# mcahny/vps

Hardware: AMD Instinct MI355X
Metric: frames/sec FuseTrack 1024x2048 (higher is better)
Workload: dtype f32-grade: f16x3 split operands (fp16 pair with scaled residual, 22 significand bits) on MFMA, f32 accumulate

## Files before the change

vps_amd/csrc/conv_mfma.hip:

```cpp
#include "conv_common.h"

namespace {
template <int TM, int TN, int WAVES_M, int WAVES_N, bool DEFORM>
__global__ __launch_bounds__(256, 2)
void conv_mfma_f32_kernel(const vps_conv_desc d, const int M, const int tiles_m, const int tiles_n,
                          const int ksteps_per_split) {
    constexpr int BN = WAVES_N * TN * 32;
    static_assert(WAVES_M * TM * 32 == BM, "block M tile must be 128");
    static_assert(WAVES_M * WAVES_N == 4, "4 wavefronts per block");
    constexpr int NB = BN / 32;

    __shared__ __attribute__((aligned(16))) float As[BM * LDS_LD];
    __shared__ __attribute__((aligned(16))) float Bs[BN * LDS_LD];

    const int t = threadIdx.x;
    int swz = xcd_swizzle(blockIdx.x, gridDim.x);
    int tile_n, tile_m, cls, split;
    decode_tile(d, swz, tiles_n, tiles_m, tile_n, tile_m, cls, split);

    const int py = cls / d.os_x, px = cls - py * d.os_x;
    const int pad_y = d.pad_y[py], pad_x = d.pad_x[px];
    const float* __restrict__ wcls = d.w + (size_t)cls * d.cout_pad * d.kpad;

    const int H = d.H, W = d.W, KH = d.KH, KW = d.KW, cin_pad = d.cin_pad;
    const int k4 = t & 7;
    const int r0 = t >> 3;

    RowInfo ri[4];
#pragma unroll
    for (int i = 0; i < 4; ++i) {
        const int m = tile_m * BM + r0 + 32 * i;
        if (m < M) {
            const int qx = m % d.Qw;
            const int tq = m / d.Qw;
            const int qy = tq % d.Qh;
            const int n = tq / d.Qh;
            ri[i].iy0 = qy * d.stride - pad_y;
            ri[i].ix0 = qx * d.stride - pad_x;
            ri[i].pixbase = n * H * W;
            ri[i].moff = m;
        } else {
            ri[i].iy0 = -(1 << 24);
            ri[i].ix0 = 0;
            ri[i].pixbase = 0;
            ri[i].moff = -1;
        }
    }

    const int kstep0 = split * ksteps_per_split;
    int nsteps = d.kpad / BK - kstep0;
    if (nsteps > ksteps_per_split) nsteps = ksteps_per_split;
    const int korder = d.korder, ntap = KH * KW;
    int ky, kx, ci;
    if (korder == 0) {
        const int kk = kstep0 * BK + k4 * 4;
        const int tap = kk / cin_pad;
        ci = kk - tap * cin_pad;
        ky = tap / KW;
        kx = tap - ky * KW;
    } else {
        const int chunk = kstep0 / ntap, tap = kstep0 - chunk * ntap;
        ci = chunk * BK + k4 * 4;
        ky = tap / KW;
        kx = tap - ky * KW;
    }
    const float* __restrict__ wrow = wcls + (size_t)(tile_n * BN + r0) * d.kpad + (size_t)kstep0 * BK + k4 * 4;

    f32x4 areg[4];
    unsigned aok = 0;
    f32x4 breg[NB];
    f32x4 dcv[DEFORM ? 4 : 1][4];
    float dcw[DEFORM ? 4 : 1][4];

    auto load_tiles = [&](int step) {
        const bool kval = ky < KH && ci < cin_pad;
        if constexpr (!DEFORM) {
#pragma unroll
            for (int i = 0; i < 4; ++i) {
                const int iy = ri[i].iy0 + ky, ix = ri[i].ix0 + kx;
                const bool ok = kval && (unsigned)iy < (unsigned)H && (unsigned)ix < (unsigned)W;
                const int pix = ri[i].pixbase + (ok ? iy * W + ix : 0);
                areg[i] = *reinterpret_cast<const f32x4*>(d.in + ((size_t)pix * d.in_ld + d.in_coff + (ok ? ci : 0)));
                aok = (aok & ~(1u << i)) | ((ok ? 1u : 0u) << i);
            }
        } else {
            const int tap = ky * KW + kx;
#pragma unroll
            for (int i = 0; i < 4; ++i) {
                const bool act = kval && ri[i].moff >= 0;
                const float* op = d.offset + (size_t)(act ? ri[i].moff : 0) * d.off_ld + 2 * min(tap, KH * KW - 1);
                const float h_im = (float)(ri[i].iy0 + ky) + op[0];
                const float w_im = (float)(ri[i].ix0 + kx) + op[1];
                const bool inside = act && h_im > -1.f && w_im > -1.f && h_im < (float)H && w_im < (float)W;
                const float hf = floorf(h_im), wf = floorf(w_im);
                const int h_low = inside ? (int)hf : 0, w_low = inside ? (int)wf : 0;
                const int h_high = h_low + 1, w_high = w_low + 1;
                const float lh = h_im - hf, lw = w_im - wf;
                const float hh = 1.f - lh, hw = 1.f - lw;
                const bool hl = inside && h_low >= 0, hhv = inside && h_high <= H - 1;
                const bool wl = w_low >= 0, whv = w_high <= W - 1;
                dcw[i][0] = (hl && wl) ? hh * hw : 0.f;
                dcw[i][1] = (hl && whv) ? hh * lw : 0.f;
                dcw[i][2] = (hhv && wl) ? lh * hw : 0.f;
                dcw[i][3] = (hhv && whv) ? lh * lw : 0.f;
                const int hlc = min(max(h_low, 0), H - 1), hhc = min(max(h_high, 0), H - 1);
                const int wlc = min(max(w_low, 0), W - 1), whc = min(max(w_high, 0), W - 1);
                const float* base = d.in + (size_t)ri[i].pixbase * d.in_ld + d.in_coff + ci;
                dcv[i][0] = *reinterpret_cast<const f32x4*>(base + (size_t)(hlc * W + wlc) * d.in_ld);
                dcv[i][1] = *reinterpret_cast<const f32x4*>(base + (size_t)(hlc * W + whc) * d.in_ld);
                dcv[i][2] = *reinterpret_cast<const f32x4*>(base + (size_t)(hhc * W + wlc) * d.in_ld);
                dcv[i][3] = *reinterpret_cast<const f32x4*>(base + (size_t)(hhc * W + whc) * d.in_ld);
            }
        }
#pragma unroll
        for (int j = 0; j < NB; ++j)
            breg[j] = *reinterpret_cast<const f32x4*>(wrow + (size_t)(32 * j) * d.kpad + (size_t)step * BK);
        if (korder == 0) {
            ci += BK;
            while (ci >= cin_pad) {
                ci -= cin_pad;
                if (++kx == KW) { kx = 0; ++ky; }
            }
        } else if (++kx == KW) {
            kx = 0;
            if (++ky == KH) { ky = 0; ci += BK; }
        }
    };

    auto store_tiles = [&]() {
#pragma unroll
        for (int i = 0; i < 4; ++i) {
            f32x4 v;
            if constexpr (DEFORM) {
                v = dcw[i][0] * dcv[i][0] + dcw[i][1] * dcv[i][1] + dcw[i][2] * dcv[i][2] + dcw[i][3] * dcv[i][3];
            } else {
                const f32x4 z = {0.f, 0.f, 0.f, 0.f};
                v = ((aok >> i) & 1u) ? areg[i] : z;
            }
            *reinterpret_cast<f32x4*>(&As[(r0 + 32 * i) * LDS_LD + k4 * 4]) = v;
        }
#pragma unroll
        for (int j = 0; j < NB; ++j)
            *reinterpret_cast<f32x4*>(&Bs[(r0 + 32 * j) * LDS_LD + k4 * 4]) = breg[j];
    };

    const int lane = t & 63, wave = t >> 6;
    const int wm = wave / WAVES_N, wn = wave - wm * WAVES_N;
    const int frag_off = (lane & 31) * LDS_LD + (lane >> 5) * 4;

    f32x16 acc[TM][TN];
#pragma unroll
    for (int a = 0; a < TM; ++a)
#pragma unroll
        for (int b = 0; b < TN; ++b)
#pragma unroll
            for (int r = 0; r < 16; ++r) acc[a][b][r] = 0.f;

    if (nsteps > 0) {
        load_tiles(0);
        store_tiles();
    }
    __syncthreads();

    for (int step = 0; step < nsteps; ++step) {
        const bool more = step + 1 < nsteps;
        if (more) load_tiles(step + 1);
#pragma unroll
        for (int kg = 0; kg < 4; ++kg) {
            f32x4 af[TM], bf[TN];
#pragma unroll
            for (int a = 0; a < TM; ++a)
                af[a] = *reinterpret_cast<const f32x4*>(&As[(wm * TM * 32 + a * 32) * LDS_LD + frag_off + kg * 8]);
#pragma unroll
            for (int b = 0; b < TN; ++b)
                bf[b] = *reinterpret_cast<const f32x4*>(&Bs[(wn * TN * 32 + b * 32) * LDS_LD + frag_off + kg * 8]);
#pragma unroll
            for (int j = 0; j < 4; ++j)
#pragma unroll
                for (int a = 0; a < TM; ++a)
#pragma unroll
                    for (int b = 0; b < TN; ++b)
                        acc[a][b] = __builtin_amdgcn_mfma_f32_32x32x2f32(bf[b][j], af[a][j], acc[a][b], 0, 0, 0);
        }
        __syncthreads();
        if (more) {
            store_tiles();
            __syncthreads();
        }
    }

    conv_epilogue<TM, TN, BN>(d, acc, M, tile_m, tile_n, cls, split, py, px, wm, wn, lane, (cls * tiles_m + tile_m) * tiles_n + tile_n);
}

template <int TM, int TN, int WAVES_M, int WAVES_N, int MODE, bool TAPMAJOR, bool DEFORM = false>
__global__ __launch_bounds__(256, (TN >= 4 ? 1 : 2))
void conv_mfma_bf16p_kernel(const vps_conv_desc d, const int M, const int tiles_m, const int tiles_n,
                            const int ksteps_per_split) {
    constexpr int BN = WAVES_N * TN * 32;
    static_assert(WAVES_M * TM * 32 == BM, "block M tile must be 128");
    static_assert(WAVES_M * WAVES_N == 4, "4 wavefronts per block");
    typedef Split<MODE> SM;
    typedef typename SM::elem elem_t;
    typedef vec8<elem_t> x8;
    typedef vec4<elem_t> x4;
    constexpr int NSA = SM::NSA, NSB = SM::NSB;
    constexpr int ABUF = NSA * BM * LDS_LDH;

    __shared__ __attribute__((aligned(16))) elem_t As[2 * ABUF];
    constexpr int DTAP = 9;
    __shared__ __attribute__((aligned(16))) float cw[DEFORM ? BM * DTAP * 4 : 4];
    __shared__ __attribute__((aligned(8))) unsigned short cc[DEFORM ? BM * DTAP * 4 : 4];
    static_assert(!(DEFORM && TAPMAJOR), "deformable layers use the chunk-major order");

    const int t = threadIdx.x;
    int swz = xcd_swizzle(blockIdx.x, gridDim.x);
    int tile_n, tile_m, cls, split;
    decode_tile(d, swz, tiles_n, tiles_m, tile_n, tile_m, cls, split);

    const int py = cls / d.os_x, px = cls - py * d.os_x;
    const int pad_y = d.pad_y[py], pad_x = d.pad_x[px];
    const int H = d.H, W = d.W, KH = d.KH, KW = d.KW, cin_pad = d.cin_pad;
    const int k4 = t & 7;
    const int r0 = t >> 3;

    RowInfo ri[4];
#pragma unroll
    for (int i = 0; i < 4; ++i) {
        const int m = tile_m * BM + r0 + 32 * i;
        if (m < M) {
            const int qx = m % d.Qw;
            const int tq = m / d.Qw;
            const int qy = tq % d.Qh;
            const int n = tq / d.Qh;
            ri[i].iy0 = qy * d.stride - pad_y;
            ri[i].ix0 = qx * d.stride - pad_x;
            ri[i].pixbase = n * H * W;
        } else {
            ri[i].iy0 = -(1 << 24);
            ri[i].ix0 = 0;
            ri[i].pixbase = 0;
        }
        ri[i].moff = m;
    }

    const int kstep0 = split * ksteps_per_split;
    int nsteps = d.kpad / BK - kstep0;
    if (nsteps > ksteps_per_split) nsteps = ksteps_per_split;
    const int korder = d.korder, ntap = KH * KW;
    int ky = 0, kx = 0, chunk = 0, astep = kstep0;
    if constexpr (!TAPMAJOR) {
        chunk = kstep0 / ntap;
        const int tap = kstep0 - chunk * ntap;
        ky = tap / KW;
        kx = tap - ky * KW;
    }
    (void)korder;

    const int lane = t & 63;
    const int wave = __builtin_amdgcn_readfirstlane(t >> 6);
    const int wm = wave / WAVES_N, wn = wave - wm * WAVES_N;
    const int nbt = d.cout_pad >> 5, kst = d.kpad >> 4;
    const size_t wplane = (size_t)d.nclass * nbt * kst * 512;
    const __amdgpu_buffer_rsrc_t wrsrc = make_rsrc(d.w_split, (unsigned)(wplane * NSB * sizeof(elem_t)));
    const unsigned wbase = (unsigned)((((size_t)(cls * nbt + tile_n * (BN / 32) + wn * TN) * kst + 2 * (size_t)kstep0) * 512) * sizeof(elem_t));
    const unsigned wlane = (unsigned)lane * 16u;
    const unsigned in_bytes = (unsigned)((size_t)d.N * H * W * d.in_ld * sizeof(float));
    const __amdgpu_buffer_rsrc_t arsrc = make_rsrc(d.in, in_bytes);
    const unsigned ld4 = (unsigned)d.in_ld * 4u;
    const unsigned acoff = (unsigned)(d.in_coff + k4 * 4) * 4u;
    unsigned rowoff[4];
#pragma unroll
    for (int i = 0; i < 4; ++i) rowoff[i] = (unsigned)(ri[i].pixbase + ri[i].iy0 * W + ri[i].ix0) * ld4 + acoff;

    f32x4 areg[DEFORM ? 1 : 2][4];
    f32x4 dcv[DEFORM ? 4 : 1][4];
    float dcw[DEFORM ? 4 : 1][4];
    x8 bnext[2][NSB][TN];
    float amax = 0.f;

    auto load_A = [&](const int slot) {
        int kyc, kxc, chunk_of_step = 0;
        unsigned stepoff;
        bool kv;
        if constexpr (!TAPMAJOR) {
            kyc = ky; kxc = kx;
            kv = chunk * BK + k4 * 4 < cin_pad;
            chunk_of_step = chunk;
            stepoff = (unsigned)(kyc * W + kxc) * ld4 + (unsigned)chunk * (BK * 4u);
            if (++kx == KW) {
                kx = 0;
                if (++ky == KH) { ky = 0; ++chunk; }
            }
        } else {
            const int kk = astep * BK + k4 * 4;
            const int tap = kk / cin_pad;
            const int cic = kk - tap * cin_pad;
            kyc = tap / KW;
            kxc = tap - kyc * KW;
            kv = tap < ntap;
            stepoff = (unsigned)(kyc * W + kxc) * ld4 + (unsigned)(cic - k4 * 4) * 4u;
        }
        ++astep;
        if constexpr (DEFORM) {
            const int tap = min(kyc * KW + kxc, DTAP - 1);
            const unsigned choff = acoff + (unsigned)chunk_of_step * (BK * 4u);
#pragma unroll
            for (int i = 0; i < 4; ++i) {
                const int e = ((r0 + 32 * i) * DTAP + tap) * 4;
                const f32x4 w4 = *reinterpret_cast<const f32x4*>(&cw[e]);
                const vec4<unsigned short> c4 = *reinterpret_cast<const vec4<unsigned short>*>(&cc[e]);
                dcw[i][0] = w4[0]; dcw[i][1] = w4[1]; dcw[i][2] = w4[2]; dcw[i][3] = w4[3];
                const unsigned pb = (unsigned)ri[i].pixbase;
                const unsigned o00 = (pb + (unsigned)c4[0] * W + c4[2]) * ld4 + choff, o01 = (pb + (unsigned)c4[0] * W + c4[3]) * ld4 + choff;
                const unsigned o10 = (pb + (unsigned)c4[1] * W + c4[2]) * ld4 + choff, o11 = (pb + (unsigned)c4[1] * W + c4[3]) * ld4 + choff;
                dcv[i][0] = buffer_load16<f32x4>(arsrc, kv ? o00 : 0xFFFFFFF0u, 0u);
                dcv[i][1] = buffer_load16<f32x4>(arsrc, kv ? o01 : 0xFFFFFFF0u, 0u);
                dcv[i][2] = buffer_load16<f32x4>(arsrc, kv ? o10 : 0xFFFFFFF0u, 0u);
                dcv[i][3] = buffer_load16<f32x4>(arsrc, kv ? o11 : 0xFFFFFFF0u, 0u);
            }
        } else {
#pragma unroll
            for (int i = 0; i < 4; ++i) {
                const int iy = ri[i].iy0 + kyc, ix = ri[i].ix0 + kxc;
                const bool ok = kv && (unsigned)iy < (unsigned)H && (unsigned)ix < (unsigned)W;
                areg[slot][i] = buffer_load16<f32x4>(arsrc, ok ? rowoff[i] + stepoff : 0xFFFFFFF0u, 0u);
            }
        }
    };

    auto load_B = [&](int step, int m, int p) {
#pragma unroll
        for (int b = 0; b < TN; ++b)
            bnext[m][p][b] = buffer_load16<x8>(wrsrc, wlane, wbase + (unsigned)(((size_t)p * wplane + ((size_t)b * kst + 2 * step + m) * 512) * sizeof(elem_t)));
    };

    auto store_A = [&](int i, int buf, const int slot) {
        x4 sp[NSA];
        if constexpr (DEFORM) split_act<MODE>(dcw[i][0] * dcv[i][0] + dcw[i][1] * dcv[i][1] + dcw[i][2] * dcv[i][2] + dcw[i][3] * dcv[i][3], sp, amax);
        else split_act<MODE>(areg[slot][i], sp, amax);
        const int row = r0 + 32 * i;
#pragma unroll
        for (int p = 0; p < NSA; ++p)
            *reinterpret_cast<x4*>(&As[buf * ABUF + p * (BM * LDS_LDH) + row * LDS_LDH + (((k4 >> 1) ^ lds_swz(row)) << 3) + ((k4 & 1) << 2)]) = sp[p];
    };

    const int frag_row = (wm * TM * 32 + (lane & 31)) * LDS_LDH;
    const int frag_sw = lds_swz(lane & 31);
    const int frag_chunk[2] = {(((lane >> 5)) ^ frag_sw) << 3, ((2 + (lane >> 5)) ^ frag_sw) << 3};
    x8 af[2][NSA][TM];
    auto read_A = [&](int m, int buf) {
#pragma unroll
        for (int p = 0; p < NSA; ++p)
#pragma unroll
            for (int a = 0; a < TM; ++a)
                af[m][p][a] = *reinterpret_cast<const x8*>(&As[buf * ABUF + p * (BM * LDS_LDH) + a * 32 * LDS_LDH + frag_row + frag_chunk[m]]);
    };

    f32x16 acc[TM][TN];
#pragma unroll
    for (int a = 0; a < TM; ++a)
#pragma unroll
        for (int b = 0; b < TN; ++b)
#pragma unroll
            for (int r = 0; r < 16; ++r) acc[a][b][r] = 0.f;

    if constexpr (DEFORM) {
        for (int e = t; e < BM * DTAP; e += 256) {
            const int row = e / DTAP, tap = e - row * DTAP;
            const int m = tile_m * BM + row;
            const bool act = m < M && tap < ntap;
            const int mm = act ? m : 0;
            const int qx = mm % d.Qw, tq = mm / d.Qw, qy = tq % d.Qh;
            const int tky = tap / KW, tkx = tap - tky * KW;
            const float* op = d.offset + (size_t)mm * d.off_ld + 2 * min(tap, ntap - 1);
            const float h_im = (float)(qy * d.stride - pad_y + tky) + op[0];
            const float w_im = (float)(qx * d.stride - pad_x + tkx) + op[1];
            const bool inside = act && h_im > -1.f && w_im > -1.f && h_im < (float)H && w_im < (float)W;
            const float hf = floorf(h_im), wf = floorf(w_im);
            const int h_low = inside ? (int)hf : 0, w_low = inside ? (int)wf : 0;
            const int h_high = h_low + 1, w_high = w_low + 1;
            const float lh = h_im - hf, lw = w_im - wf;
            const float hh = 1.f - lh, hw = 1.f - lw;
            const bool hl = inside && h_low >= 0, hhv = inside && h_high <= H - 1;
            const bool wl = w_low >= 0, whv = w_high <= W - 1;
            const f32x4 w4 = {(hl && wl) ? hh * hw : 0.f, (hl && whv) ? hh * lw : 0.f, (hhv && wl) ? lh * hw : 0.f, (hhv && whv) ? lh * lw : 0.f};
            *reinterpret_cast<f32x4*>(&cw[e * 4]) = w4;
            vec4<unsigned short> c4;
            c4[0] = (unsigned short)min(max(h_low, 0), H - 1); c4[1] = (unsigned short)min(max(h_high, 0), H - 1);
            c4[2] = (unsigned short)min(max(w_low, 0), W - 1); c4[3] = (unsigned short)min(max(w_high, 0), W - 1);
            *reinterpret_cast<vec4<unsigned short>*>(&cc[e * 4]) = c4;
        }
        __syncthreads();
    }
    if (nsteps > 0) {
        load_A(0);
#pragma unroll
        for (int m = 0; m < 2; ++m)
#pragma unroll
            for (int p = 0; p < SM::NLB; ++p) load_B(0, m, p);
#pragma unroll
        for (int i = 0; i < 4; ++i) store_A(i, 0, 0);
        if constexpr (DEFORM) {
            load_A(0);
        } else {
            load_A(1);
            load_A(0);
        }
    }
    __syncthreads();

    constexpr int NT = SM::NT;
    constexpr int NMF = 2 * NT * TM * TN;
    constexpr int NLB = SM::NLB;
    constexpr int NW = 4 + 1 + 1 + 2 * NLB;

    auto kstep = [&](const int step, auto cur_tag) {
        constexpr int cur = decltype(cur_tag)::value;
        const int bstep = min(step + 1, nsteps - 1);
        x8 bcur[2][NSB][TN];
#pragma unroll
        for (int m = 0; m < 2; ++m) {
#pragma unroll
            for (int p = 0; p < NLB; ++p)
#pragma unroll
                for (int b = 0; b < TN; ++b) bcur[m][p][b] = bnext[m][p][b];
            if constexpr (NLB < NSB) {
#pragma unroll
                for (int b = 0; b < TN; ++b) bcur[m][2][b] = derive_weight_plane<MODE>(bcur[m][0][b]);
            }
        }
        read_A(0, cur);
        __builtin_amdgcn_sched_barrier(0);

        auto work = [&](const int w) {
            constexpr int slot = DEFORM ? 0 : (cur ^ 1);
            if (w < 2) store_A(w, cur ^ 1, slot);
            else if (w == 2) read_A(1, cur);
            else if (w < 5) store_A(w - 1, cur ^ 1, slot);
            else if (w == 5) load_A(slot);
            else load_B(bstep, (w - 6) / NLB, (w - 6) % NLB);
        };

        int mf = 0;
#pragma unroll
        for (int m = 0; m < 2; ++m)
#pragma unroll
            for (int q = 0; q < NT; ++q)
#pragma unroll
                for (int a = 0; a < TM; ++a)
#pragma unroll
                    for (int b = 0; b < TN; ++b) {
                        acc[a][b] = split_mfma<MODE>(bcur[m][SM::PB[q]][b], af[m][SM::PA[q]][a], acc[a][b]);
                        ++mf;
#pragma unroll
                        for (int w = 0; w < NW; ++w) {
                            const int pos = ((w + 1) * NMF) / (NW + 1);
                            if (mf == (pos < 1 ? 1 : pos)) {
                                __builtin_amdgcn_sched_barrier(0);
                                work(w);
                                __builtin_amdgcn_sched_barrier(0);
                            }
                        }
                    }
        __syncthreads();
    };
    for (int step = 0; step < nsteps; step += 2) {
        kstep(step, std::integral_constant<int, 0>{});
        if (step + 1 < nsteps) kstep(step + 1, std::integral_constant<int, 1>{});
    }
    report_range<MODE>(d, amax);
    conv_epilogue<TM, TN, BN, false, 4, DEFORM>(d, acc, M, tile_m, tile_n, cls, split, py, px, wm, wn, lane, (cls * tiles_m + tile_m) * tiles_n + tile_n);
}

template <int TM, int TN, int WAVES_M, int WAVES_N, int MODE, int KH, int KW>
__global__ __launch_bounds__(256, 2)
void conv_mfma_bf16h_kernel(const vps_conv_desc d, const int tiles_m, const int tiles_n, const int chunks_per_split) {
    constexpr int BN = WAVES_N * TN * 32;
    static_assert(WAVES_M * TM * 32 == BM, "block M tile must be 128");
    static_assert(WAVES_M * WAVES_N == 4, "4 wavefronts per block");
    constexpr int NTAP = KH * KW;
    constexpr int HW = 16 + KW - 1, HH = 8 + KH - 1;
    constexpr int HROWS = HH * HW;
    constexpr int NLD = (HROWS + 31) / 32;
    typedef Split<MODE> SM;
    typedef typename SM::elem elem_t;
    typedef vec8<elem_t> x8;
    typedef vec4<elem_t> x4;
    constexpr int NSA = SM::NSA, NSB = SM::NSB;
    constexpr int PLANE = NLD * 32 * LDS_LDH;
    constexpr int ABUF = NSA * PLANE;

    __shared__ __attribute__((aligned(16))) elem_t As[2 * ABUF];

    const int t = threadIdx.x;
    int swz = xcd_swizzle(blockIdx.x, gridDim.x);
    int tile_n, tile_m, cls, split;
    decode_tile(d, swz, tiles_n, tiles_m, tile_n, tile_m, cls, split);

    const int py = cls / d.os_x, px = cls - py * d.os_x;
    const int H = d.H, W = d.W, cin_pad = d.cin_pad;
    const int tiles_x = (d.Qw + 15) >> 4, tiles_y = (d.Qh + 7) >> 3;
    const int tx = tile_m % tiles_x, tq = tile_m / tiles_x;
    const int ty = tq % tiles_y, n = tq / tiles_y;
    const int iy_org = ty * 8 - d.pad_y[py], ix_org = tx * 16 - d.pad_x[px];

    const int k4 = t & 7;
    const int r0 = t >> 3;
    const int chunk0 = split * chunks_per_split;
    const int nchunks = min(chunks_per_split, d.kpad / (BK * NTAP) - chunk0);
    const int nsteps = nchunks * NTAP;

    const int lane = t & 63;
    const int wave = __builtin_amdgcn_readfirstlane(t >> 6);
    const int wm = wave / WAVES_N, wn = wave - wm * WAVES_N;
    const int nbt = d.cout_pad >> 5, kst = d.kpad >> 4;
    const size_t wplane = (size_t)d.nclass * nbt * kst * 512;
    const __amdgpu_buffer_rsrc_t wrsrc = make_rsrc(d.w_split, (unsigned)(wplane * NSB * sizeof(elem_t)));
    const unsigned wbase = (unsigned)((((size_t)(cls * nbt + tile_n * (BN / 32) + wn * TN) * kst + 2 * (size_t)chunk0 * NTAP) * 512) * sizeof(elem_t));
    const unsigned wlane = (unsigned)lane * 16u;
    const __amdgpu_buffer_rsrc_t arsrc = make_rsrc(d.in, (unsigned)((size_t)d.N * H * W * d.in_ld * sizeof(float)));
    const unsigned ld4 = (unsigned)d.in_ld * 4u;

    f32x4 areg[NLD];
    int achunk = chunk0;
    x8 bnext[2][NSB][TN];
    float amax = 0.f;

    unsigned hoff[NLD];
#pragma unroll
    for (int i = 0; i < NLD; ++i) {
        const int hp = r0 + 32 * i;
        const int hy = hp / HW, hx = hp - hy * HW;
        const int iy = iy_org + hy, ix = ix_org + hx;
        const bool ok = hp < HROWS && (unsigned)iy < (unsigned)H && (unsigned)ix < (unsigned)W;
        hoff[i] = ok ? (unsigned)((n * H + iy) * W + ix) * ld4 + (unsigned)(d.in_coff + k4 * 4) * 4u : 0xFFFFFFF0u;
    }

    auto load_A = [&]() {
        const bool kv = achunk * BK + k4 * 4 < cin_pad;
        const unsigned coff = (unsigned)achunk * (BK * 4u);
        ++achunk;
#pragma unroll
        for (int i = 0; i < NLD; ++i)
            areg[i] = buffer_load16<f32x4>(arsrc, (kv && hoff[i] != 0xFFFFFFF0u) ? hoff[i] + coff : 0xFFFFFFF0u, 0u);
    };
    auto load_B = [&](int step, int m, int p) {
#pragma unroll
        for (int b = 0; b < TN; ++b)
            bnext[m][p][b] = buffer_load16<x8>(wrsrc, wlane, wbase + (unsigned)(((size_t)p * wplane + ((size_t)b * kst + 2 * step + m) * 512) * sizeof(elem_t)));
    };
    auto store_A = [&](int i, int buf) {
        x4 sp[NSA];
        split_act<MODE>(areg[i], sp, amax);
        const int row = r0 + 32 * i;
#pragma unroll
        for (int p = 0; p < NSA; ++p)
            *reinterpret_cast<x4*>(&As[buf * ABUF + p * PLANE + row * LDS_LDH + (((k4 >> 1) ^ lds_swz(row)) << 3) + ((k4 & 1) << 2)]) = sp[p];
    };

    int hbase[TM];
#pragma unroll
    for (int a = 0; a < TM; ++a) {
        const int j = wm * TM * 32 + a * 32 + (lane & 31);
        hbase[a] = (j >> 4) * HW + (j & 15);
    }
    x8 af[2][NSA][TM];
    auto read_A = [&](int m, int buf, int toff) {
#pragma unroll
        for (int a = 0; a < TM; ++a) {
            const int hrow = hbase[a] + toff;
            const int off = buf * ABUF + hrow * LDS_LDH + (((2 * m + (lane >> 5)) ^ lds_swz(hrow)) << 3);
#pragma unroll
            for (int p = 0; p < NSA; ++p) af[m][p][a] = *reinterpret_cast<const x8*>(&As[off + p * PLANE]);
        }
    };

    f32x16 acc[TM][TN];
#pragma unroll
    for (int a = 0; a < TM; ++a)
#pragma unroll
        for (int b = 0; b < TN; ++b)
#pragma unroll
            for (int r = 0; r < 16; ++r) acc[a][b][r] = 0.f;

    load_A();
#pragma unroll
    for (int m = 0; m < 2; ++m)
#pragma unroll
        for (int p = 0; p < NSB; ++p) load_B(0, m, p);
#pragma unroll
    for (int i = 0; i < NLD; ++i) store_A(i, 0);
    load_A();
    __syncthreads();

    constexpr int NT = SM::NT;
    constexpr int NMF = 2 * NT * TM * TN;
    constexpr int SPT = (NLD + NTAP - 2) / (NTAP - 1);

    for (int chunk = 0; chunk < nchunks; ++chunk) {
        const int cur = chunk & 1;
#pragma unroll
        for (int tp = 0; tp < NTAP; ++tp) {
            const int step = chunk * NTAP + tp;
            const int bstep = min(step + 1, nsteps - 1);
            const int toff = (tp / KW) * HW + (tp % KW);
            constexpr int NLB = NSB;
            x8 bcur[2][NSB][TN];
#pragma unroll
            for (int m = 0; m < 2; ++m) {
#pragma unroll
                for (int p = 0; p < NLB; ++p)
#pragma unroll
                    for (int b = 0; b < TN; ++b) bcur[m][p][b] = bnext[m][p][b];
                if constexpr (NLB < NSB) {
#pragma unroll
                    for (int b = 0; b < TN; ++b) bcur[m][2][b] = derive_weight_plane<MODE>(bcur[m][0][b]);
                }
            }
            read_A(0, cur, toff);
            __builtin_amdgcn_sched_barrier(0);

            const int NW = SPT + 1 + 2 * NLB;
            auto work = [&](const int w) {
                if (w == 1) read_A(1, cur, toff);
                else if (w == 0 || (w >= 2 && w < SPT + 1)) {
                    const int si = (w == 0 ? 0 : w - 1);
                    if (tp < NTAP - 1) {
                        const int row = tp * SPT + si;
                        if (row < NLD) store_A(row, cur ^ 1);
                    } else if (si == 0) load_A();
                } else load_B(bstep, (w - SPT - 1) / NLB, (w - SPT - 1) % NLB);
            };

            int mf = 0;
#pragma unroll
            for (int m = 0; m < 2; ++m)
#pragma unroll
                for (int q = 0; q < NT; ++q)
#pragma unroll
                    for (int a = 0; a < TM; ++a)
#pragma unroll
                        for (int b = 0; b < TN; ++b) {
                            acc[a][b] = split_mfma<MODE>(bcur[m][SM::PB[q]][b], af[m][SM::PA[q]][a], acc[a][b]);
                            ++mf;
#pragma unroll
                            for (int w = 0; w < NW; ++w) {
                                const int pos = ((w + 1) * NMF) / (NW + 1);
                                if (mf == (pos < 1 ? 1 : pos)) {
                                    __builtin_amdgcn_sched_barrier(0);
                                    work(w);
                                    __builtin_amdgcn_sched_barrier(0);
                                }
                            }
                        }
        }
        __syncthreads();
    }
    report_range<MODE>(d, amax);
    conv_epilogue<TM, TN, BN, true>(d, acc, tiles_m * BM, tile_m, tile_n, cls, split, py, px, wm, wn, lane, (cls * tiles_m + tile_m) * tiles_n + tile_n);
}

template <int V>
__global__ __launch_bounds__(256)
void conv_splitk_reduce_kernel(const vps_conv_desc d, const int M) {
    const int cv = d.cout / V;
    const size_t total = (size_t)d.nclass * M * cv;
    const size_t plane = (size_t)d.nclass * M * d.cout_pad;
    for (size_t idx = (size_t)blockIdx.x * blockDim.x + threadIdx.x; idx < total;
         idx += (size_t)gridDim.x * blockDim.x) {
        const int co = (int)(idx % cv) * V;
        const size_t t2 = idx / cv;
        const int m = (int)(t2 % M);
        const int cls = (int)(t2 / M);
        const float* __restrict__ wp = d.ws + ((size_t)cls * M + m) * d.cout_pad + co;
        float s[V];
#pragma unroll
        for (int e = 0; e < V; ++e) s[e] = 0.f;
        for (int sp0 = 0; sp0 < d.ksplit; sp0 += 8) {
            float v[8][V];
#pragma unroll
            for (int j = 0; j < 8; ++j) {
                const float* q = wp + (size_t)min(sp0 + j, d.ksplit - 1) * plane;
                if constexpr (V == 4) {
                    const f32x4 t = *reinterpret_cast<const f32x4*>(q);
                    v[j][0] = t[0]; v[j][1] = t[1]; v[j][2] = t[2]; v[j][3] = t[3];
                } else {
                    v[j][0] = q[0];
                }
            }
#pragma unroll
            for (int j = 0; j < 8; ++j)
#pragma unroll
                for (int e = 0; e < V; ++e) s[e] = (sp0 + j < d.ksplit) ? s[e] + v[j][e] : s[e];
        }
        const int py = cls / d.os_x, px = cls - py * d.os_x;
        const int qx = m % d.Qw;
        const int tq = m / d.Qw;
        const int qy = tq % d.Qh;
        const int n = tq / d.Qh;
        const int oy = qy * d.os_y + py, ox = qx * d.os_x + px;
        const size_t opix = ((size_t)n * d.Ho + oy) * d.Wo + ox;
        const int rs = d.res_shift;
        const size_t rpix = ((size_t)n * (d.Ho >> rs) + (oy >> rs)) * (d.Wo >> rs) + (ox >> rs);
        float r[V];
#pragma unroll
        for (int e = 0; e < V; ++e) r[e] = 0.f;
        if (d.res) {
            if constexpr (V == 4) {
                const f32x4 t = *reinterpret_cast<const f32x4*>(d.res + rpix * d.res_ld + d.res_coff + co);
                r[0] = t[0]; r[1] = t[1]; r[2] = t[2]; r[3] = t[3];
            } else {
                r[0] = d.res[rpix * d.res_ld + d.res_coff + co];
            }
        }
        float o[V];
#pragma unroll
        for (int e = 0; e < V; ++e) {
            float v = s[e] * (d.scale ? d.scale[co + e] : 1.f) + (d.shift ? d.shift[co + e] : 0.f);
            if (d.res) v += r[e];
            o[e] = vps_act(v, d.act, d.slope);
        }
        float* op = d.out + opix * d.out_ld + d.out_coff + co;
        if constexpr (V == 4) *reinterpret_cast<f32x4*>(op) = f32x4{o[0], o[1], o[2], o[3]};
        else op[0] = o[0];
    }
}

template <int TM, int TN, int WAVES_M, int WAVES_N>
void launch_conv(const vps_conv_desc& d, const conv_plan& p, hipStream_t s) {
    const dim3 grid(p.grid), block(p.block);
    if (p.kernel == CONV_K_HALO) {
        with_prec<true>(d.prec, [&](auto mode) {
            constexpr int MODE = decltype(mode)::value;
            if (d.KH == 3) hipLaunchKernelGGL((conv_mfma_bf16h_kernel<TM, TN, WAVES_M, WAVES_N, MODE, 3, 3>), grid, block, 0, s, d, p.tiles_m, p.tiles_n, p.chunks_per_split);
            else hipLaunchKernelGGL((conv_mfma_bf16h_kernel<TM, TN, WAVES_M, WAVES_N, MODE, 2, 2>), grid, block, 0, s, d, p.tiles_m, p.tiles_n, p.chunks_per_split);
        });
        return;
    }
#define VPS_CONV_LAUNCH(KERNEL) hipLaunchKernelGGL((KERNEL), grid, block, 0, s, d, p.M, p.tiles_m, p.tiles_n, p.per_split)
    if (p.kernel == CONV_K_F32) {
        if (d.offset) VPS_CONV_LAUNCH((conv_mfma_f32_kernel<TM, TN, WAVES_M, WAVES_N, true>));
        else VPS_CONV_LAUNCH((conv_mfma_f32_kernel<TM, TN, WAVES_M, WAVES_N, false>));
        return;
    }
    const bool tapmajor = d.korder == 0 && d.KH * d.KW > 1;
    with_prec<true>(d.prec, [&](auto mode) {
        constexpr int MODE = decltype(mode)::value;
        if (d.offset) VPS_CONV_LAUNCH((conv_mfma_bf16p_kernel<TM, TN, WAVES_M, WAVES_N, MODE, false, true>));
        else if (tapmajor) VPS_CONV_LAUNCH((conv_mfma_bf16p_kernel<TM, TN, WAVES_M, WAVES_N, MODE, true>));
        else VPS_CONV_LAUNCH((conv_mfma_bf16p_kernel<TM, TN, WAVES_M, WAVES_N, MODE, false>));
    });
#undef VPS_CONV_LAUNCH
}

conv_switches conv_switches_now(const vps_conv_desc& d) {
    const auto on = [](const char* name) { const char* const e = getenv(name); return !(e && atoi(e) == 0); };
    const auto not0 = [](const char* name) { const char* const e = getenv(name); return !(e && e[0] == '0'); };
    static const bool s2_halo = not0("VPS_S2_HALO"), thin = on("VPS_THIN"), debug_occ = getenv("VPS_DEBUG_OCC") != nullptr;
    conv_switches sw = {true, true, true, true, s2_halo, thin, debug_occ};
    if (d.prec != VPS_PREC_F16X3) return sw;
    if (d.tile_n == 32) {
        if (d.cout > 16) sw.n32 = not0("VPS_N32");
        else if (d.nclass == 4) sw.n16t = on("VPS_N16T");
    } else if (d.tile_n <= 128 && d.KH == 1) sw.pw = on("VPS_PW");
    else if (d.tile_n == 128 && d.KH == 3 && d.stride == 1) sw.h8p = on("VPS_H8P");
    return sw;
}

const conv_limits& conv_limits_once(const bool debug) {
    static const conv_limits lim = [debug] {
        conv_limits l = {};
        int dev = 0;
        (void)hipGetDevice(&dev);
        (void)hipDeviceGetAttribute(&l.cus, hipDeviceAttributeMultiprocessorCount, dev);
        vpsi_conv_pw_limits(l, debug);
        vpsi_conv_thin_limits(l, debug);
        if (debug) vpsi_conv_q_debug_occ();
        return l;
    }();
    return lim;
}

}

extern "C" int vps_conv2d(const vps_conv_desc* dp, void* stream) {
    if (!dp) return VPS_EARG(1);
    const vps_conv_desc& d = *dp;
    if (const int e = vpsi_conv_check(d)) return e;
    const conv_switches sw = conv_switches_now(d);
    const conv_plan p = vpsi_conv_plan(d, conv_limits_once(sw.debug_occ), sw);
    hipStream_t s = (hipStream_t)stream;
    switch (p.kernel) {
        case CONV_K_NONE: return p.err;
        case CONV_K_SMALL3X3V: case CONV_K_SMALL_BATCHED: case CONV_K_SMALL: vpsi_launch_conv_small(d, p, s); break;
        case CONV_K_THIN: vpsi_launch_conv_thin(d, p, s); break;
        case CONV_K_DCN256:
            hipLaunchKernelGGL((conv_mfma_bf16p_kernel<2, 4, 2, 2, VPS_PREC_F16X3, false, true>), dim3(p.grid), dim3(p.block), 0, s, d, p.M, p.tiles_m, p.tiles_n, p.per_split);
            break;
        case CONV_K_N16T: case CONV_K_N32: case CONV_K_N16: vpsi_launch_conv_n16(d, p, s); break;
        case CONV_K_H8S2: vpsi_launch_conv_h8s2(d, p, s); break;
        case CONV_K_H8P: vpsi_launch_conv_h8p(d, p, s); break;
        case CONV_K_H8: vpsi_launch_conv_h8(d, p, s); break;
        case CONV_K_PW: vpsi_launch_conv_pw(d, p, s); break;
        case CONV_K_Q: vpsi_launch_conv_q(d, p, s); break;
        default:
            if (d.tile_n == 128) launch_conv<2, 2, 2, 2>(d, p, s);
            else if (d.tile_n == 64) launch_conv<2, 1, 2, 2>(d, p, s);
            else launch_conv<1, 1, 4, 1>(d, p, s);
    }
    int st = vps_launch_status();
    if (st || !p.needs_reduce) return st;
    const size_t total = (size_t)d.nclass * p.M * d.cout;
    if (p.reduce_v4) hipLaunchKernelGGL(conv_splitk_reduce_kernel<4>, dim3(stream_grid((long)(total / 4), 256)), dim3(256), 0, s, d, p.M);
    else hipLaunchKernelGGL(conv_splitk_reduce_kernel<1>, dim3(stream_grid((long)total, 256)), dim3(256), 0, s, d, p.M);
    return vps_launch_status();
}
```

Measured before the change: 56.41.

## Tile deformable conv over 16x8 pixel patches and interleave per-row gathers

When the output dimensions divide evenly, deformable conv blocks now map their 128 output rows to a 16x8 spatial patch instead of a linear run of pixels. The aim is better cache locality for the bilinear gather loads. Sampling coordinates are precomputed into two packed byte offsets per tap (with an x-step flag bit), which removes the per-step address arithmetic. The per-row gather loads are also split out and interleaved into the k-step work schedule, optionally placing B loads first, to overlap gathers with MFMA work. This adds template variants and relies on the patch-aware epilogue path.

```diff
diff --git a/vps_amd/csrc/conv_mfma.hip b/vps_amd/csrc/conv_mfma.hip
--- a/vps_amd/csrc/conv_mfma.hip
+++ b/vps_amd/csrc/conv_mfma.hip
@@ -1,6 +1,8 @@
 #include "conv_common.h"
 
 namespace {
+typedef unsigned int u32x2 __attribute__((ext_vector_type(2)));
+
 template <int TM, int TN, int WAVES_M, int WAVES_N, bool DEFORM>
 __global__ __launch_bounds__(256, 2)
 void conv_mfma_f32_kernel(const vps_conv_desc d, const int M, const int tiles_m, const int tiles_n,
@@ -192,7 +194,7 @@
     conv_epilogue<TM, TN, BN>(d, acc, M, tile_m, tile_n, cls, split, py, px, wm, wn, lane, (cls * tiles_m + tile_m) * tiles_n + tile_n);
 }
 
-template <int TM, int TN, int WAVES_M, int WAVES_N, int MODE, bool TAPMAJOR, bool DEFORM = false>
+template <int TM, int TN, int WAVES_M, int WAVES_N, int MODE, bool TAPMAJOR, bool DEFORM = false, bool PATCH = false>
 __global__ __launch_bounds__(256, (TN >= 4 ? 1 : 2))
 void conv_mfma_bf16p_kernel(const vps_conv_desc d, const int M, const int tiles_m, const int tiles_n,
                             const int ksteps_per_split) {
@@ -209,8 +211,9 @@
     __shared__ __attribute__((aligned(16))) elem_t As[2 * ABUF];
     constexpr int DTAP = 9;
     __shared__ __attribute__((aligned(16))) float cw[DEFORM ? BM * DTAP * 4 : 4];
-    __shared__ __attribute__((aligned(8))) unsigned short cc[DEFORM ? BM * DTAP * 4 : 4];
+    __shared__ __attribute__((aligned(8))) unsigned co[DEFORM ? BM * DTAP * 2 : 2];
     static_assert(!(DEFORM && TAPMAJOR), "deformable layers use the chunk-major order");
+    static_assert(DEFORM || !PATCH, "the patch mapping is the deformable layers' (the others have the halo kernels)");
 
     const int t = threadIdx.x;
     int swz = xcd_swizzle(blockIdx.x, gridDim.x);
@@ -223,15 +226,34 @@
     const int k4 = t & 7;
     const int r0 = t >> 3;
 
+    int pt_n = 0, pt_y0 = 0, pt_x0 = 0;
+    if constexpr (PATCH) {
+        const int tiles_x = d.Qw >> 4, tiles_y = d.Qh >> 3;
+        const int tx = tile_m % tiles_x, tq = tile_m / tiles_x;
+        pt_x0 = tx << 4; pt_y0 = (tq % tiles_y) << 3; pt_n = tq / tiles_y;
+    }
+    auto row_pixel = [&](const int row, int& m, int& n, int& qy, int& qx) {
+        if constexpr (PATCH) {
+            n = pt_n; qy = pt_y0 + (row >> 4); qx = pt_x0 + (row & 15);
+            m = (n * d.Qh + qy) * d.Qw + qx;
+            return true;
+        } else {
+            m = tile_m * BM + row;
+            const bool ok = m < M;
+            const int mm = ok ? m : 0;
+            qx = mm % d.Qw;
+            const int tq = mm / d.Qw;
+            qy = tq % d.Qh;
+            n = tq / d.Qh;
+            return ok;
+        }
+    };
+
     RowInfo ri[4];
 #pragma unroll
     for (int i = 0; i < 4; ++i) {
-        const int m = tile_m * BM + r0 + 32 * i;
-        if (m < M) {
-            const int qx = m % d.Qw;
-            const int tq = m / d.Qw;
-            const int qy = tq % d.Qh;
-            const int n = tq / d.Qh;
+        int m, n, qy, qx;
+        if (row_pixel(r0 + 32 * i, m, n, qy, qx)) {
             ri[i].iy0 = qy * d.stride - pad_y;
             ri[i].ix0 = qx * d.stride - pad_x;
             ri[i].pixbase = n * H * W;
@@ -275,6 +297,7 @@
     f32x4 areg[DEFORM ? 1 : 2][4];
     f32x4 dcv[DEFORM ? 4 : 1][4];
     float dcw[DEFORM ? 4 : 1][4];
+    int dtap = 0; unsigned dchoff = 0; bool dkv = false;
     x8 bnext[2][NSB][TN];
     float amax = 0.f;
 
@@ -302,22 +325,9 @@
         }
         ++astep;
         if constexpr (DEFORM) {
-            const int tap = min(kyc * KW + kxc, DTAP - 1);
-            const unsigned choff = acoff + (unsigned)chunk_of_step * (BK * 4u);
-#pragma unroll
-            for (int i = 0; i < 4; ++i) {
-                const int e = ((r0 + 32 * i) * DTAP + tap) * 4;
-                const f32x4 w4 = *reinterpret_cast<const f32x4*>(&cw[e]);
-                const vec4<unsigned short> c4 = *reinterpret_cast<const vec4<unsigned short>*>(&cc[e]);
-                dcw[i][0] = w4[0]; dcw[i][1] = w4[1]; dcw[i][2] = w4[2]; dcw[i][3] = w4[3];
-                const unsigned pb = (unsigned)ri[i].pixbase;
-                const unsigned o00 = (pb + (unsigned)c4[0] * W + c4[2]) * ld4 + choff, o01 = (pb + (unsigned)c4[0] * W + c4[3]) * ld4 + choff;
-                const unsigned o10 = (pb + (unsigned)c4[1] * W + c4[2]) * ld4 + choff, o11 = (pb + (unsigned)c4[1] * W + c4[3]) * ld4 + choff;
-                dcv[i][0] = buffer_load16<f32x4>(arsrc, kv ? o00 : 0xFFFFFFF0u, 0u);
-                dcv[i][1] = buffer_load16<f32x4>(arsrc, kv ? o01 : 0xFFFFFFF0u, 0u);
-                dcv[i][2] = buffer_load16<f32x4>(arsrc, kv ? o10 : 0xFFFFFFF0u, 0u);
-                dcv[i][3] = buffer_load16<f32x4>(arsrc, kv ? o11 : 0xFFFFFFF0u, 0u);
-            }
+            dtap = min(kyc * KW + kxc, DTAP - 1);
+            dchoff = (unsigned)chunk_of_step * (BK * 4u);
+            dkv = kv;
         } else {
 #pragma unroll
             for (int i = 0; i < 4; ++i) {
@@ -325,6 +335,19 @@
                 const bool ok = kv && (unsigned)iy < (unsigned)H && (unsigned)ix < (unsigned)W;
                 areg[slot][i] = buffer_load16<f32x4>(arsrc, ok ? rowoff[i] + stepoff : 0xFFFFFFF0u, 0u);
             }
+        }
+    };
+
+    auto load_A_row = [&](const int i) {
+        const int e = ((r0 + 32 * i) * DTAP + dtap) * 4;
+        const f32x4 w4 = *reinterpret_cast<const f32x4*>(&cw[e]);
+        const u32x2 o2 = *reinterpret_cast<const u32x2*>(&co[e >> 1]);
+        const unsigned dx = (o2[0] & 1u) ? ld4 : 0u;
+        const unsigned o4[4] = {(o2[0] & ~1u) + acoff, (o2[0] & ~1u) + acoff + dx, o2[1] + acoff, o2[1] + acoff + dx};
+#pragma unroll
+        for (int c = 0; c < 4; ++c) {
+            dcw[i][c] = w4[c];
+            dcv[i][c] = buffer_load16<f32x4>(arsrc, dkv ? o4[c] : 0xFFFFFFF0u, dchoff);
         }
     };
 
@@ -367,10 +390,10 @@
     if constexpr (DEFORM) {
         for (int e = t; e < BM * DTAP; e += 256) {
             const int row = e / DTAP, tap = e - row * DTAP;
-            const int m = tile_m * BM + row;
-            const bool act = m < M && tap < ntap;
+            int m, n, qy, qx;
+            const bool act = row_pixel(row, m, n, qy, qx) && tap < ntap;
             const int mm = act ? m : 0;
-            const int qx = mm % d.Qw, tq = mm / d.Qw, qy = tq % d.Qh;
+            if (!act) n = qy = qx = 0;
             const int tky = tap / KW, tkx = tap - tky * KW;
             const float* op = d.offset + (size_t)mm * d.off_ld + 2 * min(tap, ntap - 1);
             const float h_im = (float)(qy * d.stride - pad_y + tky) + op[0];
@@ -385,15 +408,20 @@
             const bool wl = w_low >= 0, whv = w_high <= W - 1;
             const f32x4 w4 = {(hl && wl) ? hh * hw : 0.f, (hl && whv) ? hh * lw : 0.f, (hhv && wl) ? lh * hw : 0.f, (hhv && whv) ? lh * lw : 0.f};
             *reinterpret_cast<f32x4*>(&cw[e * 4]) = w4;
-            vec4<unsigned short> c4;
-            c4[0] = (unsigned short)min(max(h_low, 0), H - 1); c4[1] = (unsigned short)min(max(h_high, 0), H - 1);
-            c4[2] = (unsigned short)min(max(w_low, 0), W - 1); c4[3] = (unsigned short)min(max(w_high, 0), W - 1);
-            *reinterpret_cast<vec4<unsigned short>*>(&cc[e * 4]) = c4;
+            const int hlc = min(max(h_low, 0), H - 1), hhc = min(max(h_high, 0), H - 1);
+            const int wlc = min(max(w_low, 0), W - 1), whc = min(max(w_high, 0), W - 1);
+            const unsigned pb = (unsigned)(n * H * W);
+            const u32x2 o2 = {(pb + (unsigned)(hlc * W + wlc)) * ld4 | (unsigned)(whc - wlc), (pb + (unsigned)(hhc * W + wlc)) * ld4};
+            *reinterpret_cast<u32x2*>(&co[e * 2]) = o2;
         }
         __syncthreads();
     }
     if (nsteps > 0) {
         load_A(0);
+        if constexpr (DEFORM) {
+#pragma unroll
+            for (int i = 0; i < 4; ++i) load_A_row(i);
+        }
 #pragma unroll
         for (int m = 0; m < 2; ++m)
 #pragma unroll
@@ -402,6 +430,8 @@
         for (int i = 0; i < 4; ++i) store_A(i, 0, 0);
         if constexpr (DEFORM) {
             load_A(0);
+#pragma unroll
+            for (int i = 0; i < 4; ++i) load_A_row(i);
         } else {
             load_A(1);
             load_A(0);
@@ -412,7 +442,8 @@
     constexpr int NT = SM::NT;
     constexpr int NMF = 2 * NT * TM * TN;
     constexpr int NLB = SM::NLB;
-    constexpr int NW = 4 + 1 + 1 + 2 * NLB;
+    constexpr int NW = 4 + 1 + (DEFORM ? 0 : 1) + 2 * NLB;
+    constexpr bool BFIRST = DEFORM && TN >= 4;
 
     auto kstep = [&](const int step, auto cur_tag) {
         constexpr int cur = decltype(cur_tag)::value;
@@ -432,8 +463,22 @@
         read_A(0, cur);
         __builtin_amdgcn_sched_barrier(0);
 
-        auto work = [&](const int w) {
+        auto work = [&](int w) {
             constexpr int slot = DEFORM ? 0 : (cur ^ 1);
+            if constexpr (DEFORM) {
+                if constexpr (BFIRST) {
+                    const int i = w - (2 * NLB + 1);
+                    w = w == 2 ? 2 : w <= 2 * NLB ? 5 + w - (w > 2) : i < 2 ? i : i + 1;
+                }
+                if (w < 5 && w != 2) {
+                    const int i = w < 2 ? w : w - 1;
+                    store_A(i, cur ^ 1, 0);
+                    if (i == 0) load_A(0);
+                    load_A_row(i);
+                } else if (w == 2) read_A(1, cur);
+                else load_B(bstep, (w - 5) / NLB, (w - 5) % NLB);
+                return;
+            }
             if (w < 2) store_A(w, cur ^ 1, slot);
             else if (w == 2) read_A(1, cur);
             else if (w < 5) store_A(w - 1, cur ^ 1, slot);
@@ -469,7 +514,7 @@
         if (step + 1 < nsteps) kstep(step + 1, std::integral_constant<int, 1>{});
     }
     report_range<MODE>(d, amax);
-    conv_epilogue<TM, TN, BN, false, 4, DEFORM>(d, acc, M, tile_m, tile_n, cls, split, py, px, wm, wn, lane, (cls * tiles_m + tile_m) * tiles_n + tile_n);
+    conv_epilogue<TM, TN, BN, PATCH, 4, DEFORM>(d, acc, M, tile_m, tile_n, cls, split, py, px, wm, wn, lane, (cls * tiles_m + tile_m) * tiles_n + tile_n);
 }
 
 template <int TM, int TN, int WAVES_M, int WAVES_N, int MODE, int KH, int KW>
@@ -726,6 +771,8 @@
     }
 }
 
+inline bool dcn_patch(const vps_conv_desc& d) { return d.Qw % 16 == 0 && d.Qh % 8 == 0; }
+
 template <int TM, int TN, int WAVES_M, int WAVES_N>
 void launch_conv(const vps_conv_desc& d, const conv_plan& p, hipStream_t s) {
     const dim3 grid(p.grid), block(p.block);
@@ -746,7 +793,8 @@
     const bool tapmajor = d.korder == 0 && d.KH * d.KW > 1;
     with_prec<true>(d.prec, [&](auto mode) {
         constexpr int MODE = decltype(mode)::value;
-        if (d.offset) VPS_CONV_LAUNCH((conv_mfma_bf16p_kernel<TM, TN, WAVES_M, WAVES_N, MODE, false, true>));
+        if (d.offset && dcn_patch(d)) VPS_CONV_LAUNCH((conv_mfma_bf16p_kernel<TM, TN, WAVES_M, WAVES_N, MODE, false, true, true>));
+        else if (d.offset) VPS_CONV_LAUNCH((conv_mfma_bf16p_kernel<TM, TN, WAVES_M, WAVES_N, MODE, false, true>));
         else if (tapmajor) VPS_CONV_LAUNCH((conv_mfma_bf16p_kernel<TM, TN, WAVES_M, WAVES_N, MODE, true>));
         else VPS_CONV_LAUNCH((conv_mfma_bf16p_kernel<TM, TN, WAVES_M, WAVES_N, MODE, false>));
     });
@@ -795,7 +843,8 @@
         case CONV_K_SMALL3X3V: case CONV_K_SMALL_BATCHED: case CONV_K_SMALL: vpsi_launch_conv_small(d, p, s); break;
         case CONV_K_THIN: vpsi_launch_conv_thin(d, p, s); break;
         case CONV_K_DCN256:
-            hipLaunchKernelGGL((conv_mfma_bf16p_kernel<2, 4, 2, 2, VPS_PREC_F16X3, false, true>), dim3(p.grid), dim3(p.block), 0, s, d, p.M, p.tiles_m, p.tiles_n, p.per_split);
+            if (dcn_patch(d)) hipLaunchKernelGGL((conv_mfma_bf16p_kernel<2, 4, 2, 2, VPS_PREC_F16X3, false, true, true>), dim3(p.grid), dim3(p.block), 0, s, d, p.M, p.tiles_m, p.tiles_n, p.per_split);
+            else hipLaunchKernelGGL((conv_mfma_bf16p_kernel<2, 4, 2, 2, VPS_PREC_F16X3, false, true>), dim3(p.grid), dim3(p.block), 0, s, d, p.M, p.tiles_m, p.tiles_n, p.per_split);
             break;
         case CONV_K_N16T: case CONV_K_N32: case CONV_K_N16: vpsi_launch_conv_n16(d, p, s); break;
         case CONV_K_H8S2: vpsi_launch_conv_h8s2(d, p, s); break;
```

After: 56.84, median of 6. Within noise of the previous version (+0.8%).
